# AlejandroSilvestri/os1

Hardware: AMD Instinct MI355X
Metric: frames/sec extract+match, 1920x1080 @ 2000 ORB feats (higher is better)
Workload: dtype u8

## Files before the change

### os1_amd/csrc/orbfe_extractor.hip

```cpp
#include <hip/hip_runtime.h>
#include <unistd.h>
#include <sched.h>

#include <algorithm>
#include <cctype>
#include <chrono>
#include <cmath>
#include <cstdarg>
#include <cstdio>
#include <cstdlib>
#include <cstring>
#include <memory>
#include <mutex>
#include <string>
#include <thread>
#include <vector>

#include "../../include/orbfe.h"
#include "glibc_sincosf.h"
#include "host_pool.h"
#include "orbfe_internal.h"
#include "quadtree.h"

namespace orbfe {
// ... 146 lines not shown
  bool gpuQuadtree = true;
  orbfe_vocabulary* voc = nullptr;
  int vocLevelsup = 4;
  bool pendingBow = false;
  DevBuf<uint2> d_bow;
  PinBuf<uint2> h_bow;
  std::vector<std::vector<uint2>> bowKp;
  int kpPerFrameCap = 0;
  bool geomGpuQtOk = true;
  QtParams QP{};
  int selOff[kMaxLevels + 1] = {};
  int selPerFrame = 0;
  DevBuf<uint16_t> d_own;
  hipEvent_t evQt[2] = {};
  std::vector<int> frameKpBase, frameKpCount;

  int rows = 0, cols = 0, batchCap = 0;
  PyramidParams P{};
  DevBuf<uint8_t> d_tables, d_slab, d_in;
  DevBuf<ConeRange> d_coneTab, d_coneTailTab;
  ConeParams coneTail{};
  bool tailOk = false;
  int tailBase = 0, tailTile = 48;
  ConeParams cone{};
  bool coneOk = false;
  bool qtJump = true;
  int qtLdsBudget = 120 * 1024;
  int pollWaitUs = 0;
  bool zeroCopyOut = true;
  bool zeroCopyBatches = false;
  bool ingestKernel = true;
  int coneTile = 0;
  int coneMaxFrames = 2;
  DevBuf<FastCell> d_cells;
  DevBuf<uint8_t> d_zeros;
  DevBuf<uint32_t> d_cellCount, d_slots, d_cand;
  DevBuf<const uint8_t*> d_frame0;
  template <class T> struct View { T* p = nullptr; };
  DevBuf<uint8_t> d_outArena;
  PinBuf<uint8_t> h_outArena;
  size_t outArenaBytes = 0;
  View<uint32_t> d_levelStart, d_selCount, h_levelStart, h_selCount;
  View<SelKp> d_sel, h_sel;
  View<float> d_angle, h_angle;
  View<uint8_t> d_desc, h_desc;
  View<int32_t> d_m12, h_m12, d_nm, h_nm;
  bool camSet = false, camActive = false;
  CameraModel cam{};
  View<float> d_xyUn, h_xyUn;
  bool lastCam = false, submitCam = false;
  DevBuf<float> d_unTmp;
  PinBuf<float> h_unTmp;
  DevBuf<uint16_t> d_sfiOrder;
  DevBuf<int> d_sfiOrderCount;
  DevBuf<uint32_t> d_sfiPool, d_sfiPcount;
  bool pendingMatched = false;
  DevBuf<float> d_f32tmp;
  bool profileKernels = false;
  PinBuf<const uint8_t*> h_frame0;
  PinBuf<uint32_t> h_cand;
  long long inPitch = 0;
  int inFormat = ORBFE_INPUT_GRAY8, grayVariant = ORBFE_GRAY_Q15;
  int gaussVariant = ORBFE_GAUSS_ED;
  long long grayPitch = 0;
  DevBuf<uint8_t> d_gray;
  bool inLinear = false;
  int lastFrames = 0;
  int deferredFrames = 0, deferredCap = 0;
  bool deferredMatched = false;
  std::vector<OrbfeKeyPoint> defKps;
  std::vector<uint8_t> defDesc;
  std::vector<int> defN, defNm;
  std::vector<int32_t> defM12;
  std::vector<float> defXyUn;
  bool deferredCam = false;
  bool lastGpuQt = false, lastZeroCopy = false, submitZeroCopy = false;
  bool describe4 = true;
  float stageMs[5] = {0, 0, 0, 0, 0};
  hipEvent_t ev[kMaxSub][6] = {};
  double kernMs[5] = {0, 0, 0, 0, 0};
  long long kernBatches = 0, kernFrames = 0;

  struct Meta { int16_t x, y; uint8_t score, level; };
  struct Worker {
    QuadTree qt;
    std::vector<int16_t> qx, qy;
    std::vector<uint8_t> qs;
    std::vector<int> qsel;
  };
  std::unique_ptr<HostPool> pool;
  int hostThreads = 1;
  std::vector<Worker> workers;
  std::vector<std::vector<Meta>> taskOut;
  std::vector<Meta> meta;

  ~orbfe_extractor() {
    (void)hipSetDevice(device);
    for (auto& st : streams) if (st) (void)hipStreamSynchronize(st);
    d_bow.release(); h_bow.release();
    d_tables.release(); d_coneTab.release(); d_coneTailTab.release(); d_slab.release(); d_in.release(); d_cellCount.release();
    d_sfiOrder.release(); d_sfiOrderCount.release(); d_sfiPool.release(); d_sfiPcount.release();
    d_cells.release(); d_zeros.release(); d_slots.release(); d_cand.release(); d_frame0.release(); d_gray.release(); d_outArena.release(); h_outArena.release();
    d_f32tmp.release(); d_unTmp.release(); h_unTmp.release();
    h_frame0.release(); h_cand.release();
    for (auto& es : ev) for (auto& e : es) if (e) (void)hipEventDestroy(e);
    for (auto& e : evS1) if (e) (void)hipEventDestroy(e);
    for (auto& e : evQt) if (e) (void)hipEventDestroy(e);
    d_own.release();
    if (evFrame0) (void)hipEventDestroy(evFrame0);
    if (evUpload) (void)hipEventDestroy(evUpload);

    for (auto& st : streams) if (st) (void)hipStreamDestroy(st);
  }

  int setGeometry(int r, int c) {
    if (r == rows && c == cols) return ORBFE_OK;
    if (c > 4095 || r > 4095) {
      set_err("image %dx%d exceeds the 4095-pixel coordinate packing limit", c, r);
      return ORBFE_ERR_INVALID;
    }
    bool qtOk = true;
    int kpSum = 8;
    PyramidParams Q{};
    Q.nlevels = nlevels;
    Q.iniTh = iniTh;
    Q.minTh = minTh;
    long long off = 0, slot = 0;
    int cellBase = 0;
    size_t tableBytes = 0;
    for (int l = 0; l < nlevels; l++) {
      LevelGeom& L = Q.lv[l];
      L.w = cv_round_f((float)c * isf[l]);
      L.h = cv_round_f((float)r * isf[l]);
      const float width = (float)((L.w - kEdge + 3) - (kEdge - 3));
      const float height = (float)((L.h - kEdge + 3) - (kEdge - 3));
      L.nCols = (int)(width / 30.f);
      L.nRows = (int)(height / 30.f);
      if (L.nCols < 1 || L.nRows < 1) {
        set_err("image %dx%d too small: level %d (%dx%d) has no FAST cell", c, r, l, L.w, L.h);
        return ORBFE_ERR_TOO_SMALL;
      }
      L.wCell = (int)std::ceil(width / L.nCols);
      L.hCell = (int)std::ceil(height / L.nRows);
      {
        const int nIni = (int)roundf(static_cast<float>(L.w - 2 * kBorder) / (L.h - 2 * kBorder));
        if (nIni < 1 || nIni > 4) qtOk = false;
        kpSum += std::max(nfeat[l] + 4, 4 * std::max(nIni, 4));
      }
      L.cellBase = cellBase;
      cellBase += L.nCols * L.nRows;
      L.slotCap = (((L.wCell + 1) / 2) * ((L.hCell + 1) / 2) + 3) & ~3;
      L.slotBase = slot;
      slot += (long long)L.nCols * L.nRows * L.slotCap;
      if (l >= 1) {
// ... 422 lines not shown
    float* angOut = zeroCopy ? h_angle.p : d_angle.p;
    uint8_t* descOut = zeroCopy ? h_desc.p : d_desc.p;
    const int qtLds = small ? qtLdsBudget : 0;
    const bool four = describe4 && small;
    const bool localCand = small && localLists;
    submitLocalCand = localCand;
    QP.levelLocal = localCand ? 1 : 0;
    {
      if (prof) HIP_TRY(hipEventRecord(ev[0][0], st));
      if (launch_pyramid(P, nframes, st, coneOk && small ? &cone : (tailOk && !small ? &coneTail : nullptr))) { set_err("cannot configure the pyramid kernel"); return ORBFE_ERR_HIP; }
      const bool timeFast = prof || !small;
      fastTimed = timeFast;
      if (timeFast) HIP_TRY(hipEventRecord(ev[0][1], st));
      launch_fast(P, nframes, st);
      if (timeFast) HIP_TRY(hipEventRecord(ev[0][2], st));
      if (localCand) launch_compact_local(P, nframes, st, 0, nlevels);
      else launch_compact(P, nframes, st);
      if (prof) HIP_TRY(hipEventRecord(ev[0][3], st));
      if (prof) HIP_TRY(hipEventRecord(evQt[0], st));
      if (launch_quadtree(QP, nframes, st, qtLds)) { set_err("cannot configure the quadtree kernel"); return ORBFE_ERR_HIP; }
      if (prof) HIP_TRY(hipEventRecord(evQt[1], st));
      if (prof) HIP_TRY(hipEventRecord(ev[0][4], st));
      launch_describe_slots(P, d_sel.p, nframes * selPerFrame, angOut, descOut, d_selCount.p, selPerFrame, selOff, st, four,
                            kernelOut ? h_angle.p : nullptr, kernelOut ? h_desc.p : nullptr);
      if (prof) HIP_TRY(hipEventRecord(ev[0][5], st));
      HIP_TRY(hipGetLastError());
    }
    const int nslots = nframes * selPerFrame;
    submitCam = camActive;
    if (camActive) {
      UndistortArgs U{};
      U.cam = cam; U.in = nullptr; U.sel = d_sel.p; U.selCount = d_selCount.p;
      U.out = zeroCopy ? h_xyUn.p : d_xyUn.p;
      U.n = nslots; U.selPerFrame = selPerFrame; U.nlevels = nlevels;
      for (int l = 0; l <= nlevels; l++) U.selOff[l] = selOff[l];
      for (int l = 0; l < nlevels; l++) U.sf[l] = sf[l];
      launch_undistort(U, st);
      HIP_TRY(hipGetLastError());
      if (kernelOut) HIP_TRY(hipMemcpyAsync(h_xyUn.p, d_xyUn.p, 2 * sizeof(float) * (size_t)nslots, hipMemcpyDeviceToHost, st));
    }
    pendingBow = false;
    if (voc) {
      if ((rc = d_bow.ensure(nslots)) || (rc = h_bow.ensure(nslots))) return rc;
      if ((rc = bow_launch_descend(voc, d_desc.p, nslots, vocLevelsup, d_bow.p, st))) return rc;
      HIP_TRY(hipMemcpyAsync(h_bow.p, d_bow.p, sizeof(uint2) * nslots, hipMemcpyDeviceToHost, st));
      pendingBow = true;
    }
    pendingMatched = false;
    if (ms && ms->chain) {
      orbfe_sfi_chain& ch = *ms->chain;
      const int n0cap = selOff[1] - selOff[0];
      if (ch.n0cap != n0cap || ch.device != device) { set_err("match chain belongs to a different extractor configuration"); return ORBFE_ERR_INVALID; }
      if ((rc = d_sfiOrder.ensure((size_t)batchCap * n0cap))) return rc;
      if ((rc = d_sfiOrderCount.ensure(batchCap))) return rc;
      if ((rc = d_sfiPool.ensure((size_t)batchCap * n0cap * n0cap))) return rc;
      if ((rc = d_sfiPcount.ensure((size_t)batchCap * n0cap))) return rc;
      SfiParams SP{};
      SP.sel = d_sel.p; SP.angle = d_angle.p; SP.desc = d_desc.p; SP.selCount = d_selCount.p;
      SP.selPerFrame = selPerFrame; SP.n0cap = n0cap; SP.frameBase = 0;
      const int prev = (int)((ch.seq + 1) & 1), cur = (int)(ch.seq & 1);
      SP.carrySel = ch.sel[prev].p; SP.carryAngle = ch.angle[prev].p; SP.carryDesc = ch.desc[prev].p;
      const bool iso = ch.isolated;
      if (camActive) {
        for (int i = 0; i < 2; i++)
          if ((rc = ch.xyUn[i].ensure(2 * (size_t)n0cap))) return rc;
      }
      if (ch.camera != camActive && ch.seq > 0) ch.restart = true;
      ch.camera = camActive;
      SP.xyUn = camActive ? d_xyUn.p : nullptr;
      SP.carryXyUn = camActive ? ch.xyUn[prev].p : nullptr;
      SP.carryCount = ch.count.p + ((ch.seq == 0 || iso || ch.restart) ? 2 : prev);
      ch.restart = false;
      SP.minX = ms->bounds[0]; SP.minY = ms->bounds[2];
      SP.invW = static_cast<float>(64) / static_cast<float>(ms->bounds[1] - ms->bounds[0]);
      SP.invH = static_cast<float>(48) / static_cast<float>(ms->bounds[3] - ms->bounds[2]);
      SP.window = (float)ms->window; SP.nnratio = ms->nnratio; SP.checkOri = ms->checkOri;
      SP.order = d_sfiOrder.p; SP.orderCount = d_sfiOrderCount.p; SP.pool = d_sfiPool.p; SP.pcount = d_sfiPcount.p;
      SP.matches12 = kernelOut ? h_m12.p : d_m12.p; SP.nmatches = kernelOut ? h_nm.p : d_nm.p;
      if (ch.seq > 0 && !iso) HIP_TRY(hipStreamWaitEvent(st, ch.ready[prev], 0));
      launch_sfi(SP, nframes, st);
      HIP_TRY(hipGetLastError());
      if (!iso) {
        launch_sfi_carry(SP, nframes - 1, ch.sel[cur].p, ch.angle[cur].p, ch.desc[cur].p, ch.count.p + cur, camActive ? ch.xyUn[cur].p : nullptr, st);
        HIP_TRY(hipGetLastError());
        HIP_TRY(hipEventRecord(ch.ready[cur], st));
      }
      ch.seq++;
      pendingMatched = true;
    }
    if (!zeroCopy && !kernelOut) HIP_TRY(hipMemcpyAsync(h_outArena.p, d_outArena.p, outArenaBytes, hipMemcpyDeviceToHost, st));
    submitProfiled = prof;
    tSubmit0 = t0;
    tSubmit1 = now_ms();
    pendingFrames = nframes;
    return ORBFE_OK;
  }

  int waitOnly() {
    if (!pendingFrames) return ORBFE_OK;
    HIP_TRY(hipSetDevice(device));
    hipStream_t st = streams[0];
    if (pollWaitUs > 0) {
      hipError_t q;
      while ((q = hipStreamQuery(st)) == hipErrorNotReady) usleep((useconds_t)pollWaitUs);
      if (q != hipSuccess) HIP_TRY(q);
    }
    HIP_TRY(hipStreamSynchronize(st));
    return ORBFE_OK;
  }

  int waitGpuQt(OrbfeKeyPoint* kps, uint8_t* desc, int cap, int* n_out, int32_t* matches12 = nullptr,
                int* nmatches = nullptr, float* xy_un = nullptr) {
    if (!pendingFrames) { set_err("no submitted batch to collect"); return ORBFE_ERR_INVALID; }
    HIP_TRY(hipSetDevice(device));
    const int nframes = pendingFrames;
    pendingFrames = 0;
    hipStream_t st = streams[0];
    const double t0 = tSubmit0, t1 = tSubmit1;
    const double t1b = now_ms();
    if (pollWaitUs > 0) {
      hipError_t q;
      while ((q = hipStreamQuery(st)) == hipErrorNotReady) usleep((useconds_t)pollWaitUs);
      if (q != hipSuccess) HIP_TRY(q);
    }
    HIP_TRY(hipStreamSynchronize(st));
    const double t2 = now_ms();
    {
      float ms = 0;
      if (fastTimed && hipEventElapsedTime(&ms, ev[0][1], ev[0][2]) == hipSuccess) kernMs[1] += ms;
      if (submitProfiled) {
// ... 1104 lines not shown
```

### os1_amd/csrc/orbfe_fast.hip

```cpp
#include <hip/hip_runtime.h>

#include <algorithm>
#include <cstdlib>
#include <type_traits>
#include <vector>

#include "orbfe_internal.h"

namespace orbfe {

namespace {
__device__ __forceinline__ int m24(int a, int b) { return __mul24(a, b); }
typedef unsigned short u16x2 __attribute__((ext_vector_type(2)));
__device__ __forceinline__ u16x2 as_u16x2(unsigned v) { return __builtin_bit_cast(u16x2, v); }
__device__ __forceinline__ unsigned as_u32(u16x2 v) { return __builtin_bit_cast(unsigned, v); }
}

__device__ __forceinline__ unsigned pk_min3_h(unsigned a, unsigned b, unsigned c) {
  unsigned r;
  asm("v_pk_minimum3_f16 %0, %1, %2, %3" : "=v"(r) : "v"(a), "v"(b), "v"(c));
  return r;
}
__device__ __forceinline__ unsigned pk_max3_h(unsigned a, unsigned b, unsigned c) {
  unsigned r;
// ... 131 lines not shown
    const int total = rw * rh;
    for (int i0 = lane; i0 < total; i0 += 64 * 8) {
      uint8_t v[8];
#pragma unroll
      for (int u = 0; u < 8; u++) {
        const int i = i0 + u * 64;
        v[u] = 0;
        if (i < total) {
          const int y = (int)(((float)i + 0.5f) * rcpRw), x = i - m24(y, rw);
          v[u] = roi[m24(y, istr) + x];
        }
      }
#pragma unroll
      for (int u = 0; u < 8; u++) {
        const int i = i0 + u * 64;
        if (i < total) {
          const int y = (int)(((float)i + 0.5f) * rcpRw), x = i - m24(y, rw);
          tile[m24(y, TP) + a + x] = v[u];
        }
      }
    }
  }
  tile += a;
  if constexpr (LEAN) {
    const int pieces = (SP * (eh + 2) + 15) >> 4;
#pragma nounroll
    for (int p0 = 0; p0 < pieces; p0 += 64)
      if (lane < pieces - p0)
        __builtin_amdgcn_global_load_lds((const __attribute__((address_space(1))) void*)P.zeros,
                                         (__attribute__((address_space(3))) void*)(sc + 16 * p0), 16, 0, 0);
  } else {
    const int pieces = (SP * (eh + 2) + 15) >> 4;
    for (int p0 = 0; p0 < pieces; p0 += 64)
      if (lane < pieces - p0)
        __builtin_amdgcn_global_load_lds((const __attribute__((address_space(1))) void*)P.zeros,
                                         (__attribute__((address_space(3))) void*)(sc + 16 * p0), 16, 0, 0);
  }
  asm volatile("s_waitcnt vmcnt(0)" ::: "memory");
  wave_lds_fence();
  if constexpr (ABL == 4) stamp[2] = __builtin_amdgcn_s_memtime();
  if constexpr (ABL == 1) {
    unsigned acc = 0;
    for (int i = lane; i < (TP * rh) >> 2; i += 64) acc ^= reinterpret_cast<const uint32_t*>(tile - a)[i];
    if (acc == 0x9e3779b9u && lane == 63) cnt[0] = 0;
    if (lane == 0) cnt[0] = 0;
    return;
  }

  const unsigned long long below = (1ull << lane) - 1ull;
  uint32_t* slot;
  if constexpr (LEAN) slot = reinterpret_cast<uint32_t*>(reinterpret_cast<uint8_t*>(P.slots) + 4u * ((uint32_t)f * (uint32_t)P.slotsPerFrame + slotOff));
  else slot = P.slots + (long long)f * P.slotsPerFrame + slotOff;
  int base = 0;
  for (int pass = 0; pass < 2; pass++) {
    const int tlo = pass ? P.minTh : P.iniTh;
    int nq = 0;
    constexpr int NPX = 16, GS = 4, NS = 4;
    const int G = (ew + NPX - 1) >> GS, nItems = G * eh;
    const int stepY = (int)((0x10152040u >> ((G - 1) << 3)) & 0xffu), stepG = 64 - stepY * G;
    auto stage1 = [&](auto aTag) {
      constexpr int A = decltype(aTag)::value;
      const u16x2 T2 = as_u16x2((unsigned)tlo * 0x01000100u);
      auto test4 = [&](uint32_t L4, uint32_t C4, uint32_t R4, uint32_t U4, uint32_t D4, unsigned& fe, unsigned& fo) {
        unsigned flag[2];
#pragma unroll
        for (int h = 0; h < 2; h++) {
          const u16x2 v2 = h ? as_u16x2(C4) << 8 : as_u16x2(C4);
          const u16x2 r0 = h ? as_u16x2(D4) << 8 : as_u16x2(D4), r4 = h ? as_u16x2(R4) << 8 : as_u16x2(R4);
          const u16x2 r8 = h ? as_u16x2(U4) << 8 : as_u16x2(U4), r12 = h ? as_u16x2(L4) << 8 : as_u16x2(L4);
          const u16x2 mx = __builtin_elementwise_min(__builtin_elementwise_max(r0, r8), __builtin_elementwise_max(r4, r12));
          const u16x2 mn = __builtin_elementwise_max(__builtin_elementwise_min(r0, r8), __builtin_elementwise_min(r4, r12));
          const u16x2 dd = __builtin_elementwise_max(__builtin_elementwise_sub_sat(mx, v2), __builtin_elementwise_sub_sat(v2, mn));
          const unsigned e = as_u32(__builtin_elementwise_sub_sat(dd, T2));
          asm("v_pk_min_u16 %0, %1, %2" : "=v"(flag[h]) : "v"(e), "v"(0x00010001u));
        }
        fo = flag[0];
        fe = flag[1];
      };
      int y = (int)(((float)lane + 0.5f) * __builtin_amdgcn_rcpf((float)G)), g = lane - m24(y, G);
      int ro = m24(y, TP) + (g << GS);
      const int roStep = m24(stepY, TP) + (stepG << GS), roCarry = TP - (G << GS);
      const uint8_t* tb = tile - a;
      for (int i0 = 0; i0 < nItems; i0 += 64) {
        unsigned m = 0;
        if (i0 + lane < nItems) {
          constexpr int c0 = (A + 3) >> 2, cs = (A + 3) & 3, q0 = (A + 6) >> 2, qs = (A + 6) & 3;
          const uint32_t* cw = reinterpret_cast<const uint32_t*>(tb + 3 * TP + ro);
          uint32_t w[NS + 3];
#pragma unroll
          for (int k = 0; k < NS + 3; k++) w[k] = cw[k];
          const uint32_t* uw = reinterpret_cast<const uint32_t*>(tb + ro) + c0;
          const uint32_t* dw = reinterpret_cast<const uint32_t*>(tb + 6 * TP + ro) + c0;
          uint32_t u[NS + 1], d[NS + 1];
#pragma unroll
          for (int k = 0; k < NS + 1; k++) { u[k] = uw[k]; d[k] = dw[k]; }
          unsigned E = 0, O = 0;
#pragma unroll
          for (int j = 0; j < NS; j++) {
            const uint32_t Lj = __builtin_amdgcn_alignbyte(w[j + 1], w[j], A);
            const uint32_t Cj = __builtin_amdgcn_alignbyte(w[c0 + j + 1], w[c0 + j], cs);
            const uint32_t Rj = __builtin_amdgcn_alignbyte(w[q0 + j + 1], w[q0 + j], qs);
            const uint32_t Uj = __builtin_amdgcn_alignbyte(u[j + 1], u[j], cs);
            const uint32_t Dj = __builtin_amdgcn_alignbyte(d[j + 1], d[j], cs);
            unsigned fe, fo;
            test4(Lj, Cj, Rj, Uj, Dj, fe, fo);
            E |= fe << (4 * j);
            O |= fo << (4 * j);
          }
          const unsigned T = E | (O << 1);
          const int rem = ew - (g << GS);
          m = (T | (T >> 14)) & ((1u << min(rem, NPX)) - 1u);
        }
        const int c = __popc(m);
        int incl = c;
        incl += __builtin_amdgcn_update_dpp(0, incl, 0x111, 0xf, 0xf, true);
        incl += __builtin_amdgcn_update_dpp(0, incl, 0x112, 0xf, 0xf, true);
        incl += __builtin_amdgcn_update_dpp(0, incl, 0x114, 0xf, 0xf, true);
        incl += __builtin_amdgcn_update_dpp(0, incl, 0x118, 0xf, 0xf, true);
        incl += __builtin_amdgcn_update_dpp(0, incl, 0x142, 0xa, 0xf, false);
        incl += __builtin_amdgcn_update_dpp(0, incl, 0x143, 0xc, 0xf, false);
        const int pos = nq + incl - c;
        const unsigned e = (unsigned)((y << 8) | (g << GS));
        {
          unsigned rev = __builtin_bitreverse32(m), ent = e;
          unsigned addr = (unsigned)(uintptr_t)(queue + pos);
          unsigned long long saved;
          asm volatile(
              "s_mov_b64 %3, exec\n\t"
              ".rept %4\n\t"
              "v_add_co_u32 %0, vcc, %0, %0\n\t"
              "s_and_b64 exec, %3, vcc\n\t"
              "ds_write_b16 %1, %2\n\t"
              "v_add_u32 %1, 2, %1\n\t"
              "s_mov_b64 exec, %3\n\t"
              "v_add_u32 %2, 1, %2\n\t"
              ".endr"
              : "+v"(rev), "+v"(addr), "+v"(ent), "=&s"(saved)
              : "n"(NPX)
              : "vcc", "scc", "memory");
        }
        nq += __builtin_amdgcn_readlane(incl, 63);
        if (i0 + 64 >= nItems) break;
        y += stepY;
        g += stepG;
        ro += roStep;
        if (g >= G) { g -= G; y++; ro += roCarry; }
      }
    };
    switch (a) {
      case 0: stage1(std::integral_constant<int, 0>{}); break;
      case 1: stage1(std::integral_constant<int, 1>{}); break;
      case 2: stage1(std::integral_constant<int, 2>{}); break;
      default: stage1(std::integral_constant<int, 3>{}); break;
    }
    wave_lds_fence();
    if constexpr (ABL == 4) { if (pass == 0) stamp[3] = __builtin_amdgcn_s_memtime(); }
    if constexpr (ABL == 2) {
      unsigned acc = 0;
      for (int i = lane; i < nq; i += 64) acc ^= queue[i];
      if (lane == 0) cnt[0] = (acc == 0xffffffffu) ? 1u : 0u;
      return;
    }
    int nq2 = 0;
    for (int i0 = 0; i0 < nq; i0 += 64) {
      const int i = i0 + lane;
      bool ok = false;
      unsigned e = 0;
      if (i < nq) {
        e = queue[i];
        const int y = e >> 8, x = e & 0xff;
        const uint8_t* c = tile + m24(y + 3, TP) + (x + 3);
        const unsigned vv = c[0];
        constexpr unsigned B = 2048u;
        unsigned xr[16];
        const unsigned VV = (B + vv) | ((B - vv) << 16);
#define RING(k, off) asm("v_pk_mad_i16 %0, %1, %2, %3 op_sel_hi:[0,1,1]" : "=v"(xr[k]) : "v"((unsigned)c[off]), "v"(0x0001ffffu), "v"(VV));
        RING(0, 3 * TP);       RING(1, 3 * TP + 1);   RING(2, 2 * TP + 2);    RING(3, TP + 3);
        RING(4, 3);            RING(5, -TP + 3);      RING(6, -2 * TP + 2);   RING(7, -3 * TP + 1);
        RING(8, -3 * TP);      RING(9, -3 * TP - 1);  RING(10, -2 * TP - 2);  RING(11, -TP - 3);
        RING(12, -3);          RING(13, TP - 3);      RING(14, 2 * TP - 2);   RING(15, 3 * TP - 1);
#undef RING
        unsigned t[16], arc[16];
#pragma unroll
        for (int k = 0; k < 16; k++) t[k] = pk_min3_h(xr[k], xr[(k + 1) & 15], xr[(k + 2) & 15]);
#pragma unroll
        for (int k = 0; k < 16; k++) arc[k] = pk_min3_h(t[k], t[(k + 3) & 15], t[(k + 6) & 15]);
        const unsigned m0 = pk_max3_h(arc[0], arc[1], arc[2]), m1 = pk_max3_h(arc[3], arc[4], arc[5]), m2 = pk_max3_h(arc[6], arc[7], arc[8]);
        const unsigned m3 = pk_max3_h(arc[9], arc[10], arc[11]), m4 = pk_max3_h(arc[12], arc[13], arc[14]);
        const unsigned best = pk_max3_h(pk_max3_h(m0, m1, m2), pk_max3_h(m3, m4, arc[15]), arc[15]);
        const int S = (int)max(best & 0xffffu, best >> 16) - (int)B;
        ok = S > tlo;
        if (ok) sc[m24(y + 1, SP) + (x + 1)] = (uint8_t)(S - 1);
      }
      const unsigned long long mk = __ballot(ok);
      if (ok) queue[nq2 + __popcll(mk & below)] = (uint16_t)e;
      nq2 += __popcll(mk);
    }
    wave_lds_fence();
    if constexpr (ABL == 4) { if (pass == 0) stamp[4] = __builtin_amdgcn_s_memtime(); }
    if constexpr (ABL == 3) {
      unsigned acc = 0;
      for (int i = lane; i < nq2; i += 64) acc ^= queue[i] ^ sc[i];
      if (lane == 0) cnt[0] = (acc == 0xffffffffu) ? 1u : 0u;
      return;
    }
    for (int i0 = 0; i0 < nq2; i0 += 64) {
// ... 135 lines not shown
```

### os1_amd/csrc/orbfe_internal.h

```cpp
#pragma once
#include <cstddef>
#include <cstdint>

namespace orbfe {

constexpr int kMaxLevels = 12;
constexpr int kEdge = 19;
constexpr int kBorder = 16;
constexpr int kHalfPatch = 15;
constexpr int kBlurRad = 18;
constexpr int kRawRad = kBlurRad + 3;

struct LevelGeom {
  int w, h;
  int pitch;
  long long off;
  int nCols, nRows;
  int wCell, hCell;
  int cellBase;
  int slotCap;
  long long slotBase;
  const int* xofs;
  const short* xalpha;
  const int* yofs;
// ... 46 lines not shown
  int offB, offH, offC, coefLen;
  int ldsBytes;
  const ConeRange* regX;
  const ConeRange* regY;
};

#ifdef ORBFE_EXPERIMENTS
#define ORBFE_EXP_ENV(name) getenv(name)
#else
#define ORBFE_EXP_ENV(name) (static_cast<const char*>(nullptr))
#endif
#ifdef __HIPCC__
__device__ __forceinline__ const uint8_t* level0_of(const PyramidParams& P, int f) {
  const uint8_t* p = P.frame0 ? P.frame0[f] : P.frameInline[f & 1];
  const unsigned long long v = reinterpret_cast<unsigned long long>(p);
  const unsigned lo = __builtin_amdgcn_readfirstlane((unsigned)v), hi = __builtin_amdgcn_readfirstlane((unsigned)(v >> 32));
  return reinterpret_cast<const uint8_t*>(((unsigned long long)hi << 32) | lo);
}
#endif

struct SelKp {
  uint32_t xy;
  uint32_t lf;
};

struct ExtractView {
  const SelKp* sel;
  const float* angle;
  const uint8_t* desc;
  const float* xyUn;
  int selOff[kMaxLevels + 1];
  int count[kMaxLevels];
  float sf[kMaxLevels];
  int nlevels, n, device;
  void* stream;
};

struct SfiParams {
  const SelKp* sel;
  const float* angle;
  const uint8_t* desc;
  const uint32_t* selCount;
  int selPerFrame, n0cap, frameBase;
  const SelKp* carrySel;
  const float* carryAngle;
  const uint8_t* carryDesc;
  const uint32_t* carryCount;
  const float* xyUn;
  const float* carryXyUn;
  float minX, minY, invW, invH;
  float window, nnratio;
  int checkOri;
  uint16_t* order;
  int* orderCount;
  uint32_t* pool;
  uint32_t* pcount;
  int32_t* matches12;
  int32_t* nmatches;
};

struct CameraModel {
  double fx, fy, cx, cy, ifx, ify;
  double k[8];
};
struct UndistortArgs {
  CameraModel cam;
  const float* in;
  const SelKp* sel;
  const uint32_t* selCount;
  float* out;
  int n, selPerFrame, nlevels;
  int selOff[kMaxLevels + 1];
  float sf[kMaxLevels];
};

constexpr int kQtNodeCap = 2048;

struct QtParams {
  const uint32_t* cand;
  const uint32_t* levelStart;
  long long candCap;
  int nlevels, frameBase;
  int levW[kMaxLevels], levH[kMaxLevels], nfeat[kMaxLevels];
  int selOff[kMaxLevels];
  int selPerFrame;
  uint16_t* own;
  SelKp* sel;
  uint32_t* selCount;
  SelKp* selHost;
  uint32_t* selCountHost;
  int jump;
  int levelLocal;
  long long candBase[kMaxLevels];
};


}
```

### os1_amd/csrc/orbfe_sfi.hip

```cpp
#include <hip/hip_runtime.h>

#include <cstdlib>

#include "orbfe_internal.h"

namespace orbfe {

constexpr int kSfiGridCols = 64, kSfiGridRows = 48;
constexpr int kSfiThLow = 50, kSfiHisto = 30;

struct SfiFrame {
  const float2* xyUn;
  const SelKp* sel;
  const float* angle;
  const uint8_t* desc;
  int n;
};

__device__ __forceinline__ SfiFrame sfi_frame(const SfiParams& S, int f) {
  SfiFrame F;
  if (f < 0) {
    F.sel = S.carrySel; F.angle = S.carryAngle; F.desc = S.carryDesc;
    F.xyUn = reinterpret_cast<const float2*>(S.carryXyUn);
    F.n = S.carryCount ? (int)*S.carryCount : -1;
// ... 18 lines not shown
__global__ __launch_bounds__(256) void k_sfi_sort(SfiParams S) {
  constexpr int kCells = kSfiGridCols * kSfiGridRows, kPer = kCells / 256;
  static_assert(kCells % 256 == 0, "cells per thread");
  extern __shared__ int dyn[];
  int* cellOf = dyn;
  int* arrival = dyn + S.n0cap;
  int* bucket = dyn + 2 * S.n0cap;
  __shared__ int start[kCells + 1];
  __shared__ int wsum[4];
  const int f = S.frameBase + blockIdx.x, tid = threadIdx.x;
  const SfiFrame F = sfi_frame(S, f);
  for (int c = tid; c <= kCells; c += 256) start[c] = 0;
  __syncthreads();
  for (int k = tid; k < F.n; k += 256) {
    const float2 p = sfi_pos<UN>(F, k);
    const float x = p.x, y = p.y;
    const int px = (int)roundf((x - S.minX) * S.invW), py = (int)roundf((y - S.minY) * S.invH);
    const int c = (px < 0 || px >= kSfiGridCols || py < 0 || py >= kSfiGridRows) ? -1 : px * kSfiGridRows + py;
    cellOf[k] = c;
    if (c >= 0) arrival[k] = atomicAdd(&start[c], 1);
  }
  __syncthreads();
  int loc[kPer], sum = 0;
#pragma unroll
  for (int i = 0; i < kPer; i++) { loc[i] = start[tid * kPer + i]; sum += loc[i]; }
  int incl = sum;
#pragma unroll
  for (int o = 1; o < 64; o <<= 1) {
    const int t = __shfl_up(incl, o, 64);
    if ((tid & 63) >= o) incl += t;
  }
  if ((tid & 63) == 63) wsum[tid >> 6] = incl;
  __syncthreads();
  int base = incl - sum;
  for (int w = 0; w < (tid >> 6); w++) base += wsum[w];
#pragma unroll
  for (int i = 0; i < kPer; i++) { start[tid * kPer + i] = base; base += loc[i]; }
  if (tid == 255) start[kCells] = base;
  __syncthreads();
  for (int k = tid; k < F.n; k += 256) {
    const int c = cellOf[k];
    if (c >= 0) bucket[start[c] + arrival[k]] = k;
  }
  __syncthreads();
  uint16_t* order = S.order + (long long)f * S.n0cap;
  for (int k = tid; k < F.n; k += 256) {
    const int c = cellOf[k];
    if (c < 0) continue;
    const int b0 = start[c], b1 = start[c + 1];
    int rank = 0;
    for (int j = b0; j < b1; j++) rank += bucket[j] < k;
    order[b0 + rank] = (uint16_t)k;
  }
  if (tid == 0) S.orderCount[f] = start[kCells];
}

template <bool UN>
__global__ __launch_bounds__(64) void k_sfi_candidates(SfiParams S) {
  const int i1 = blockIdx.x, fr = blockIdx.y, lane = threadIdx.x;
  const int f = S.frameBase + fr;
  const SfiFrame F2 = sfi_frame(S, f);
  const SfiFrame F1 = sfi_frame(S, fr == 0 ? -1 : f - 1);
  uint32_t* cnt = S.pcount + (long long)f * S.n0cap + i1;
  if (F1.n < 0 || i1 >= F1.n) {
    if (lane == 0 && i1 < S.n0cap) *cnt = 0;
    return;
  }
  const float2 q = sfi_pos<UN>(F1, i1);
  const float x = q.x, y = q.y, r = S.window;
  int cx0 = 0, cx1 = kSfiGridCols - 1, cy0 = 0, cy1 = kSfiGridRows - 1;
  if (UN) {
    cx0 = max(0, (int)floorf((x - S.minX - r) * S.invW));
    cx1 = min(kSfiGridCols - 1, (int)ceilf((x - S.minX + r) * S.invW));
    cy0 = max(0, (int)floorf((y - S.minY - r) * S.invH));
    cy1 = min(kSfiGridRows - 1, (int)ceilf((y - S.minY + r) * S.invH));
    if (cx0 >= kSfiGridCols || cx1 < 0 || cy0 >= kSfiGridRows || cy1 < 0) {
      if (lane == 0) *cnt = 0;
      return;
    }
  }
  uint32_t qd[8];
  const uint32_t* qp = reinterpret_cast<const uint32_t*>(F1.desc + (long long)i1 * 32);
#pragma unroll
  for (int w = 0; w < 8; w++) qd[w] = qp[w];
  const uint16_t* order = S.order + (long long)f * S.n0cap;
  const int nin = S.orderCount[f];
  uint32_t* pool = S.pool + ((long long)f * S.n0cap + i1) * S.n0cap;
  const unsigned long long below = (1ull << lane) - 1ull;
  int run = 0;
  for (int e0 = 0; e0 < nin; e0 += 64) {
    const int e = e0 + lane;
    bool ok = false;
    int i2 = 0;
    if (e < nin) {
      i2 = order[e];
      const float2 p = sfi_pos<UN>(F2, i2);
      const float dx = p.x - x, dy = p.y - y;
      ok = fabsf(dx) < r && fabsf(dy) < r;
      if (UN) {
        const int px = (int)roundf((p.x - S.minX) * S.invW), py = (int)roundf((p.y - S.minY) * S.invH);
        ok = ok && px >= cx0 && px <= cx1 && py >= cy0 && py <= cy1;
      }
    }
    const unsigned long long m = __ballot(ok);
    if (ok) {
      const uint32_t* dp = reinterpret_cast<const uint32_t*>(F2.desc + (long long)i2 * 32);
      int d = 0;
#pragma unroll
      for (int w = 0; w < 8; w++) d += __popc(dp[w] ^ qd[w]);
      pool[run + __popcll(m & below)] = (uint32_t)i2 | ((uint32_t)d << 16);
    }
    run += __popcll(m);
  }
  if (lane == 0) *cnt = (uint32_t)run;
}

__device__ __forceinline__ int sfi_rot_bin(float a1, float a2) {
  const float factor = 1.0f / kSfiHisto;
  float rot = a1 - a2;
  if (rot < 0.0f) rot += 360.0f;
  int bin = (int)roundf(rot * factor);
  if (bin == kSfiHisto) bin = 0;
  return bin;
}


__device__ int* g_sfiDbg;
constexpr int kSfiDbgRecords = 1 << 16;

template <class PoolAt>
__device__ void sfi_serial_outcomes(int lane, int n1, const int* pcnt, PoolAt poolAt, float nnratio, int* vmd, int* M) {
  for (int i1 = 0; i1 < n1; i1++) {
    const int cnt = pcnt[i1];
    int bestDist = 0x7fffffff, bestDist2 = 0x7fffffff, bestIdx2 = -1;
    for (int c0 = 0; c0 < cnt; c0 += 64) {
      int d = 0x7fffffff, i2 = -1;
      if (c0 + lane < cnt) {
        const uint32_t entry = poolAt(i1, c0 + lane);
        i2 = (int)(entry & 0xffff);
        const int dist = (int)(entry >> 16);
        if (!(vmd[i2] <= dist)) d = dist;
      }
      const unsigned dd = (d == 0x7fffffff) ? 511u : (unsigned)d;
      unsigned long long c1 = ~0ull;
#pragma unroll
      for (int b = 8; b >= 0; b--) {
        const unsigned long long z = __ballot(((dd >> b) & 1u) == 0u) & c1;
        if (z) c1 = z;
      }
      const int ml = (int)__builtin_ctzll(c1);
      const unsigned d1 = (unsigned)__shfl((int)dd, ml, 64);
      unsigned long long c2 = ~(1ull << ml);
#pragma unroll
      for (int b = 8; b >= 0; b--) {
        const unsigned long long z = __ballot(((dd >> b) & 1u) == 0u) & c2;
// ... 258 lines not shown
```

Measured before the change: 89670.

## Restrict SFI candidate scan to grid cells and cache FAST dilation between passes

The SFI candidate kernel now stores per-cell start offsets and has each query scan only the column segments of grid cells covering its search window, instead of walking every ordered keypoint. A wave prefix sum over column lengths maps each lane to its source index. Separately, the FAST stage-1 kernel keeps the per-pixel contrast values from pass 0 in registers and reapplies only the lower threshold in pass 1 when a single iteration covers all items, skipping the reload and recompute. These are unrelated changes, and the distorted path now always applies cell bounds, which may alter candidate ordering or semantics.

```diff
diff --git a/os1_amd/csrc/orbfe_extractor.hip b/os1_amd/csrc/orbfe_extractor.hip
--- a/os1_amd/csrc/orbfe_extractor.hip
+++ b/os1_amd/csrc/orbfe_extractor.hip
@@ -222,7 +222,7 @@
   DevBuf<float> d_unTmp;
   PinBuf<float> h_unTmp;
   DevBuf<uint16_t> d_sfiOrder;
-  DevBuf<int> d_sfiOrderCount;
+  DevBuf<int> d_sfiCellStart;
   DevBuf<uint32_t> d_sfiPool, d_sfiPcount;
   bool pendingMatched = false;
   DevBuf<float> d_f32tmp;
@@ -269,7 +269,7 @@
     for (auto& st : streams) if (st) (void)hipStreamSynchronize(st);
     d_bow.release(); h_bow.release();
     d_tables.release(); d_coneTab.release(); d_coneTailTab.release(); d_slab.release(); d_in.release(); d_cellCount.release();
-    d_sfiOrder.release(); d_sfiOrderCount.release(); d_sfiPool.release(); d_sfiPcount.release();
+    d_sfiOrder.release(); d_sfiCellStart.release(); d_sfiPool.release(); d_sfiPcount.release();
     d_cells.release(); d_zeros.release(); d_slots.release(); d_cand.release(); d_frame0.release(); d_gray.release(); d_outArena.release(); h_outArena.release();
     d_f32tmp.release(); d_unTmp.release(); h_unTmp.release();
     h_frame0.release(); h_cand.release();
@@ -798,7 +798,7 @@
       const int n0cap = selOff[1] - selOff[0];
       if (ch.n0cap != n0cap || ch.device != device) { set_err("match chain belongs to a different extractor configuration"); return ORBFE_ERR_INVALID; }
       if ((rc = d_sfiOrder.ensure((size_t)batchCap * n0cap))) return rc;
-      if ((rc = d_sfiOrderCount.ensure(batchCap))) return rc;
+      if ((rc = d_sfiCellStart.ensure((size_t)batchCap * (64 * 48 + 1)))) return rc;
       if ((rc = d_sfiPool.ensure((size_t)batchCap * n0cap * n0cap))) return rc;
       if ((rc = d_sfiPcount.ensure((size_t)batchCap * n0cap))) return rc;
       SfiParams SP{};
@@ -821,7 +821,7 @@
       SP.invW = static_cast<float>(64) / static_cast<float>(ms->bounds[1] - ms->bounds[0]);
       SP.invH = static_cast<float>(48) / static_cast<float>(ms->bounds[3] - ms->bounds[2]);
       SP.window = (float)ms->window; SP.nnratio = ms->nnratio; SP.checkOri = ms->checkOri;
-      SP.order = d_sfiOrder.p; SP.orderCount = d_sfiOrderCount.p; SP.pool = d_sfiPool.p; SP.pcount = d_sfiPcount.p;
+      SP.order = d_sfiOrder.p; SP.cellStart = d_sfiCellStart.p; SP.pool = d_sfiPool.p; SP.pcount = d_sfiPcount.p;
       SP.matches12 = kernelOut ? h_m12.p : d_m12.p; SP.nmatches = kernelOut ? h_nm.p : d_nm.p;
       if (ch.seq > 0 && !iso) HIP_TRY(hipStreamWaitEvent(st, ch.ready[prev], 0));
       launch_sfi(SP, nframes, st);
diff --git a/os1_amd/csrc/orbfe_fast.hip b/os1_amd/csrc/orbfe_fast.hip
--- a/os1_amd/csrc/orbfe_fast.hip
+++ b/os1_amd/csrc/orbfe_fast.hip
@@ -207,106 +207,113 @@
   if constexpr (LEAN) slot = reinterpret_cast<uint32_t*>(reinterpret_cast<uint8_t*>(P.slots) + 4u * ((uint32_t)f * (uint32_t)P.slotsPerFrame + slotOff));
   else slot = P.slots + (long long)f * P.slotsPerFrame + slotOff;
   int base = 0;
+  unsigned kd[8] = {0u, 0u, 0u, 0u, 0u, 0u, 0u, 0u};
   for (int pass = 0; pass < 2; pass++) {
     const int tlo = pass ? P.minTh : P.iniTh;
     int nq = 0;
     constexpr int NPX = 16, GS = 4, NS = 4;
     const int G = (ew + NPX - 1) >> GS, nItems = G * eh;
     const int stepY = (int)((0x10152040u >> ((G - 1) << 3)) & 0xffu), stepG = 64 - stepY * G;
-    auto stage1 = [&](auto aTag) {
+    const u16x2 T2 = as_u16x2((unsigned)tlo * 0x01000100u);
+    const bool reuse = pass == 1 && nItems <= 64;
+    auto window4 = [&](uint32_t L4, uint32_t C4, uint32_t R4, uint32_t U4, uint32_t D4, unsigned& de, unsigned& dod) {
+      unsigned dw[2];
+#pragma unroll
+      for (int h = 0; h < 2; h++) {
+        const u16x2 v2 = h ? as_u16x2(C4) << 8 : as_u16x2(C4);
+        const u16x2 r0 = h ? as_u16x2(D4) << 8 : as_u16x2(D4), r4 = h ? as_u16x2(R4) << 8 : as_u16x2(R4);
+        const u16x2 r8 = h ? as_u16x2(U4) << 8 : as_u16x2(U4), r12 = h ? as_u16x2(L4) << 8 : as_u16x2(L4);
+        const u16x2 mx = __builtin_elementwise_min(__builtin_elementwise_max(r0, r8), __builtin_elementwise_max(r4, r12));
+        const u16x2 mn = __builtin_elementwise_max(__builtin_elementwise_min(r0, r8), __builtin_elementwise_min(r4, r12));
+        dw[h] = as_u32(__builtin_elementwise_max(__builtin_elementwise_sub_sat(mx, v2), __builtin_elementwise_sub_sat(v2, mn)));
+      }
+      dod = dw[0];
+      de = dw[1];
+    };
+    const uint8_t* tb = tile - a;
+    auto words = [&](auto aTag, int ro) {
       constexpr int A = decltype(aTag)::value;
-      const u16x2 T2 = as_u16x2((unsigned)tlo * 0x01000100u);
-      auto test4 = [&](uint32_t L4, uint32_t C4, uint32_t R4, uint32_t U4, uint32_t D4, unsigned& fe, unsigned& fo) {
-        unsigned flag[2];
-#pragma unroll
-        for (int h = 0; h < 2; h++) {
-          const u16x2 v2 = h ? as_u16x2(C4) << 8 : as_u16x2(C4);
-          const u16x2 r0 = h ? as_u16x2(D4) << 8 : as_u16x2(D4), r4 = h ? as_u16x2(R4) << 8 : as_u16x2(R4);
-          const u16x2 r8 = h ? as_u16x2(U4) << 8 : as_u16x2(U4), r12 = h ? as_u16x2(L4) << 8 : as_u16x2(L4);
-          const u16x2 mx = __builtin_elementwise_min(__builtin_elementwise_max(r0, r8), __builtin_elementwise_max(r4, r12));
-          const u16x2 mn = __builtin_elementwise_max(__builtin_elementwise_min(r0, r8), __builtin_elementwise_min(r4, r12));
-          const u16x2 dd = __builtin_elementwise_max(__builtin_elementwise_sub_sat(mx, v2), __builtin_elementwise_sub_sat(v2, mn));
-          const unsigned e = as_u32(__builtin_elementwise_sub_sat(dd, T2));
-          asm("v_pk_min_u16 %0, %1, %2" : "=v"(flag[h]) : "v"(e), "v"(0x00010001u));
+      constexpr int c0 = (A + 3) >> 2, cs = (A + 3) & 3, q0 = (A + 6) >> 2, qs = (A + 6) & 3;
+      const uint32_t* cw = reinterpret_cast<const uint32_t*>(tb + 3 * TP + ro);
+      uint32_t w[NS + 3];
+#pragma unroll
+      for (int k = 0; k < NS + 3; k++) w[k] = cw[k];
+      const uint32_t* uw = reinterpret_cast<const uint32_t*>(tb + ro) + c0;
+      const uint32_t* dw = reinterpret_cast<const uint32_t*>(tb + 6 * TP + ro) + c0;
+      uint32_t u[NS + 1], d[NS + 1];
+#pragma unroll
+      for (int k = 0; k < NS + 1; k++) { u[k] = uw[k]; d[k] = dw[k]; }
+#pragma unroll
+      for (int j = 0; j < NS; j++) {
+        const uint32_t Lj = __builtin_amdgcn_alignbyte(w[j + 1], w[j], A);
+        const uint32_t Cj = __builtin_amdgcn_alignbyte(w[c0 + j + 1], w[c0 + j], cs);
+        const uint32_t Rj = __builtin_amdgcn_alignbyte(w[q0 + j + 1], w[q0 + j], qs);
+        const uint32_t Uj = __builtin_amdgcn_alignbyte(u[j + 1], u[j], cs);
+        const uint32_t Dj = __builtin_amdgcn_alignbyte(d[j + 1], d[j], cs);
+        window4(Lj, Cj, Rj, Uj, Dj, kd[2 * j + 1], kd[2 * j]);
+      }
+    };
+    int y = (int)(((float)lane + 0.5f) * __builtin_amdgcn_rcpf((float)G)), g = lane - m24(y, G);
+    int ro = m24(y, TP) + (g << GS);
+    const int roStep = m24(stepY, TP) + (stepG << GS), roCarry = TP - (G << GS);
+    for (int i0 = 0; i0 < nItems; i0 += 64) {
+      unsigned m = 0;
+      if (i0 + lane < nItems) {
+        if (!reuse) {
+          switch (a) {
+            case 0: words(std::integral_constant<int, 0>{}, ro); break;
+            case 1: words(std::integral_constant<int, 1>{}, ro); break;
+            case 2: words(std::integral_constant<int, 2>{}, ro); break;
+            default: words(std::integral_constant<int, 3>{}, ro); break;
+          }
         }
-        fo = flag[0];
-        fe = flag[1];
-      };
-      int y = (int)(((float)lane + 0.5f) * __builtin_amdgcn_rcpf((float)G)), g = lane - m24(y, G);
-      int ro = m24(y, TP) + (g << GS);
-      const int roStep = m24(stepY, TP) + (stepG << GS), roCarry = TP - (G << GS);
-      const uint8_t* tb = tile - a;
-      for (int i0 = 0; i0 < nItems; i0 += 64) {
-        unsigned m = 0;
-        if (i0 + lane < nItems) {
-          constexpr int c0 = (A + 3) >> 2, cs = (A + 3) & 3, q0 = (A + 6) >> 2, qs = (A + 6) & 3;
-          const uint32_t* cw = reinterpret_cast<const uint32_t*>(tb + 3 * TP + ro);
-          uint32_t w[NS + 3];
-#pragma unroll
-          for (int k = 0; k < NS + 3; k++) w[k] = cw[k];
-          const uint32_t* uw = reinterpret_cast<const uint32_t*>(tb + ro) + c0;
-          const uint32_t* dw = reinterpret_cast<const uint32_t*>(tb + 6 * TP + ro) + c0;
-          uint32_t u[NS + 1], d[NS + 1];
-#pragma unroll
-          for (int k = 0; k < NS + 1; k++) { u[k] = uw[k]; d[k] = dw[k]; }
-          unsigned E = 0, O = 0;
-#pragma unroll
-          for (int j = 0; j < NS; j++) {
-            const uint32_t Lj = __builtin_amdgcn_alignbyte(w[j + 1], w[j], A);
-            const uint32_t Cj = __builtin_amdgcn_alignbyte(w[c0 + j + 1], w[c0 + j], cs);
-            const uint32_t Rj = __builtin_amdgcn_alignbyte(w[q0 + j + 1], w[q0 + j], qs);
-            const uint32_t Uj = __builtin_amdgcn_alignbyte(u[j + 1], u[j], cs);
-            const uint32_t Dj = __builtin_amdgcn_alignbyte(d[j + 1], d[j], cs);
-            unsigned fe, fo;
-            test4(Lj, Cj, Rj, Uj, Dj, fe, fo);
-            E |= fe << (4 * j);
-            O |= fo << (4 * j);
-          }
-          const unsigned T = E | (O << 1);
-          const int rem = ew - (g << GS);
-          m = (T | (T >> 14)) & ((1u << min(rem, NPX)) - 1u);
+        unsigned E = 0, O = 0;
+#pragma unroll
+        for (int j = 0; j < NS; j++) {
+          unsigned fo, fe;
+          asm("v_pk_min_u16 %0, %1, %2" : "=v"(fo) : "v"(as_u32(__builtin_elementwise_sub_sat(as_u16x2(kd[2 * j]), T2))), "v"(0x00010001u));
+          asm("v_pk_min_u16 %0, %1, %2" : "=v"(fe) : "v"(as_u32(__builtin_elementwise_sub_sat(as_u16x2(kd[2 * j + 1]), T2))), "v"(0x00010001u));
+          E |= fe << (4 * j);
+          O |= fo << (4 * j);
         }
-        const int c = __popc(m);
-        int incl = c;
-        incl += __builtin_amdgcn_update_dpp(0, incl, 0x111, 0xf, 0xf, true);
-        incl += __builtin_amdgcn_update_dpp(0, incl, 0x112, 0xf, 0xf, true);
-        incl += __builtin_amdgcn_update_dpp(0, incl, 0x114, 0xf, 0xf, true);
-        incl += __builtin_amdgcn_update_dpp(0, incl, 0x118, 0xf, 0xf, true);
-        incl += __builtin_amdgcn_update_dpp(0, incl, 0x142, 0xa, 0xf, false);
-        incl += __builtin_amdgcn_update_dpp(0, incl, 0x143, 0xc, 0xf, false);
-        const int pos = nq + incl - c;
-        const unsigned e = (unsigned)((y << 8) | (g << GS));
-        {
-          unsigned rev = __builtin_bitreverse32(m), ent = e;
-          unsigned addr = (unsigned)(uintptr_t)(queue + pos);
-          unsigned long long saved;
-          asm volatile(
-              "s_mov_b64 %3, exec\n\t"
-              ".rept %4\n\t"
-              "v_add_co_u32 %0, vcc, %0, %0\n\t"
-              "s_and_b64 exec, %3, vcc\n\t"
-              "ds_write_b16 %1, %2\n\t"
-              "v_add_u32 %1, 2, %1\n\t"
-              "s_mov_b64 exec, %3\n\t"
-              "v_add_u32 %2, 1, %2\n\t"
-              ".endr"
-              : "+v"(rev), "+v"(addr), "+v"(ent), "=&s"(saved)
-              : "n"(NPX)
-              : "vcc", "scc", "memory");
-        }
-        nq += __builtin_amdgcn_readlane(incl, 63);
-        if (i0 + 64 >= nItems) break;
-        y += stepY;
-        g += stepG;
-        ro += roStep;
-        if (g >= G) { g -= G; y++; ro += roCarry; }
-      }
-    };
-    switch (a) {
-      case 0: stage1(std::integral_constant<int, 0>{}); break;
-      case 1: stage1(std::integral_constant<int, 1>{}); break;
-      case 2: stage1(std::integral_constant<int, 2>{}); break;
-      default: stage1(std::integral_constant<int, 3>{}); break;
+        const unsigned T = E | (O << 1);
+        const int rem = ew - (g << GS);
+        m = (T | (T >> 14)) & ((1u << min(rem, NPX)) - 1u);
+      }
+      const int c = __popc(m);
+      int incl = c;
+      incl += __builtin_amdgcn_update_dpp(0, incl, 0x111, 0xf, 0xf, true);
+      incl += __builtin_amdgcn_update_dpp(0, incl, 0x112, 0xf, 0xf, true);
+      incl += __builtin_amdgcn_update_dpp(0, incl, 0x114, 0xf, 0xf, true);
+      incl += __builtin_amdgcn_update_dpp(0, incl, 0x118, 0xf, 0xf, true);
+      incl += __builtin_amdgcn_update_dpp(0, incl, 0x142, 0xa, 0xf, false);
+      incl += __builtin_amdgcn_update_dpp(0, incl, 0x143, 0xc, 0xf, false);
+      const int pos = nq + incl - c;
+      const unsigned e = (unsigned)((y << 8) | (g << GS));
+      {
+        unsigned rev = __builtin_bitreverse32(m), ent = e;
+        unsigned addr = (unsigned)(uintptr_t)(queue + pos);
+        unsigned long long saved;
+        asm volatile(
+            "s_mov_b64 %3, exec\n\t"
+            ".rept %4\n\t"
+            "v_add_co_u32 %0, vcc, %0, %0\n\t"
+            "s_and_b64 exec, %3, vcc\n\t"
+            "ds_write_b16 %1, %2\n\t"
+            "v_add_u32 %1, 2, %1\n\t"
+            "s_mov_b64 exec, %3\n\t"
+            "v_add_u32 %2, 1, %2\n\t"
+            ".endr"
+            : "+v"(rev), "+v"(addr), "+v"(ent), "=&s"(saved)
+            : "n"(NPX)
+            : "vcc", "scc", "memory");
+      }
+      nq += __builtin_amdgcn_readlane(incl, 63);
+      if (i0 + 64 >= nItems) break;
+      y += stepY;
+      g += stepG;
+      ro += roStep;
+      if (g >= G) { g -= G; y++; ro += roCarry; }
     }
     wave_lds_fence();
     if constexpr (ABL == 4) { if (pass == 0) stamp[3] = __builtin_amdgcn_s_memtime(); }
diff --git a/os1_amd/csrc/orbfe_internal.h b/os1_amd/csrc/orbfe_internal.h
--- a/os1_amd/csrc/orbfe_internal.h
+++ b/os1_amd/csrc/orbfe_internal.h
@@ -122,7 +122,7 @@
   float window, nnratio;
   int checkOri;
   uint16_t* order;
-  int* orderCount;
+  int* cellStart;
   uint32_t* pool;
   uint32_t* pcount;
   int32_t* matches12;
diff --git a/os1_amd/csrc/orbfe_sfi.hip b/os1_amd/csrc/orbfe_sfi.hip
--- a/os1_amd/csrc/orbfe_sfi.hip
+++ b/os1_amd/csrc/orbfe_sfi.hip
@@ -94,7 +94,8 @@
     for (int j = b0; j < b1; j++) rank += bucket[j] < k;
     order[b0 + rank] = (uint16_t)k;
   }
-  if (tid == 0) S.orderCount[f] = start[kCells];
+  int* cellStart = S.cellStart + (long long)f * (kCells + 1);
+  for (int c = tid; c <= kCells; c += 256) cellStart[c] = start[c];
 }
 
 template <bool UN>
@@ -110,39 +111,55 @@
   }
   const float2 q = sfi_pos<UN>(F1, i1);
   const float x = q.x, y = q.y, r = S.window;
-  int cx0 = 0, cx1 = kSfiGridCols - 1, cy0 = 0, cy1 = kSfiGridRows - 1;
-  if (UN) {
-    cx0 = max(0, (int)floorf((x - S.minX - r) * S.invW));
-    cx1 = min(kSfiGridCols - 1, (int)ceilf((x - S.minX + r) * S.invW));
-    cy0 = max(0, (int)floorf((y - S.minY - r) * S.invH));
-    cy1 = min(kSfiGridRows - 1, (int)ceilf((y - S.minY + r) * S.invH));
-    if (cx0 >= kSfiGridCols || cx1 < 0 || cy0 >= kSfiGridRows || cy1 < 0) {
-      if (lane == 0) *cnt = 0;
-      return;
-    }
+  const int cx0 = max(0, (int)floorf((x - S.minX - r) * S.invW));
+  const int cx1 = min(kSfiGridCols - 1, (int)ceilf((x - S.minX + r) * S.invW));
+  const int cy0 = max(0, (int)floorf((y - S.minY - r) * S.invH));
+  const int cy1 = min(kSfiGridRows - 1, (int)ceilf((y - S.minY + r) * S.invH));
+  if (cx0 >= kSfiGridCols || cx1 < 0 || cy0 >= kSfiGridRows || cy1 < 0 || cx1 < cx0 || cy1 < cy0) {
+    if (lane == 0) *cnt = 0;
+    return;
   }
   uint32_t qd[8];
   const uint32_t* qp = reinterpret_cast<const uint32_t*>(F1.desc + (long long)i1 * 32);
 #pragma unroll
   for (int w = 0; w < 8; w++) qd[w] = qp[w];
   const uint16_t* order = S.order + (long long)f * S.n0cap;
-  const int nin = S.orderCount[f];
+  const int ncols = __builtin_amdgcn_readfirstlane(cx1 - cx0 + 1);
+  const int* cellStart = S.cellStart + (long long)f * (kSfiGridCols * kSfiGridRows + 1);
+  int rs = 0, len = 0;
+  if (lane < ncols) {
+    const int c = (cx0 + lane) * kSfiGridRows;
+    rs = cellStart[c + cy0];
+    len = cellStart[c + cy1 + 1] - rs;
+  }
+  int incl = len;
+#pragma unroll
+  for (int o = 1; o < 64; o <<= 1) {
+    const int t = __shfl_up(incl, o, 64);
+    if (lane >= o) incl += t;
+  }
+  const int first = incl - len;
+  const int shift = rs - first;
+  const int nin = __builtin_amdgcn_readlane(incl, 63);
   uint32_t* pool = S.pool + ((long long)f * S.n0cap + i1) * S.n0cap;
   const unsigned long long below = (1ull << lane) - 1ull;
   int run = 0;
   for (int e0 = 0; e0 < nin; e0 += 64) {
     const int e = e0 + lane;
+    int sh = 0;
+    for (int c = 0; c < ncols; c++) {
+      const int fc = __builtin_amdgcn_readlane(first, c);
+      if (fc >= e0 + 64) break;
+      const int sc = __builtin_amdgcn_readlane(shift, c);
+      if (e >= fc) sh = sc;
+    }
     bool ok = false;
     int i2 = 0;
     if (e < nin) {
-      i2 = order[e];
+      i2 = order[e + sh];
       const float2 p = sfi_pos<UN>(F2, i2);
       const float dx = p.x - x, dy = p.y - y;
       ok = fabsf(dx) < r && fabsf(dy) < r;
-      if (UN) {
-        const int px = (int)roundf((p.x - S.minX) * S.invW), py = (int)roundf((p.y - S.minY) * S.invH);
-        ok = ok && px >= cx0 && px <= cx1 && py >= cy0 && py <= cy1;
-      }
     }
     const unsigned long long m = __ballot(ok);
     if (ok) {
```

After: 90590, median of 6. 1.01x the previous value.
